# luigifcruz/radio-core

Measured on AMD Instinct MI355X. Metric: IQ Msamples/s through Tuner+WBFM at 1024 channels, higher is better.
Workload: dtype f32

## Files before the change

### radio-core_amd/csrc/fft_kernel.h

```cpp
#pragma once

#include <hip/hip_runtime.h>

#include <cstdio>
#include <cstdlib>
#include <type_traits>

#include "fft_engine.h"
#include "tile_ns.h"

namespace rcfm {
RCFM_NS_OPEN
namespace fftk {

constexpr int W = RCFM_TILE_W;
constexpr int kLogW = W == 16 ? 4 : W == 8 ? 3 : 2;
static_assert((1 << kLogW) == W, "tile width: 4, 8 or 16 lines");
constexpr int kThreads = 256 * W / 16;

__device__ __forceinline__ float2 cmul(float2 a, float2 b) {
    typedef float v2f __attribute__((ext_vector_type(2)));
    v2f A, B, D;
    A.x = a.x; A.y = a.y; B.x = b.x; B.y = b.y;
    asm("v_pk_mul_f32 %0, %1, %2 op_sel:[0,0] op_sel_hi:[0,1]" : "=v"(D) : "v"(A), "v"(B));
// ... 171 lines not shown
    dft5(v[0], v[2], v[4], v[6], v[8]);
    dft5(v[1], v[3], v[5], v[7], v[9]);
    v[3] = cmul(v[3], make_float2(0.80901699437494742410f, -0.58778525229247312917f));
    v[5] = cmul(v[5], make_float2(0.30901699437494742410f, -0.95105651629515357212f));
    v[7] = cmul(v[7], make_float2(-0.30901699437494742410f, -0.95105651629515357212f));
    v[9] = cmul(v[9], make_float2(-0.80901699437494742410f, -0.58778525229247312917f));
    dft2(v[0], v[1]);
    dft2(v[2], v[3]);
    dft2(v[4], v[5]);
    dft2(v[6], v[7]);
    dft2(v[8], v[9]);
    const float2 y0 = v[0], y5 = v[1], y1 = v[2], y6 = v[3], y2 = v[4], y7 = v[5], y3 = v[6], y8 = v[7],
                 y4 = v[8], y9 = v[9];
    v[0] = y0; v[1] = y1; v[2] = y2; v[3] = y3; v[4] = y4;
    v[5] = y5; v[6] = y6; v[7] = y7; v[8] = y8; v[9] = y9;
}

template <int R>
__device__ __forceinline__ void dif_stage(float2* tile, const float2* tw, int L, int mt, int swz) {
    const int m = mt / R;
    const int step = L / mt;
    const int nb = (L / R) * W;
    for (int e = threadIdx.x; e < nb; e += kThreads) {
        const int w = e & (W - 1);
        const int b = e / W;
        const int g = b / m;
        const int kp = b - g * m;
        const int base = g * mt + kp;
        float2 v[R];
#pragma unroll
        for (int q = 0; q < R; ++q) {
            const int row = base + q * m;
            v[q] = tile[row * W + (w ^ (swz & row & (W - 1)))];
        }
        if constexpr (R == 2) dft2(v[0], v[1]);
        if constexpr (R == 3) dft3(v[0], v[1], v[2]);
        if constexpr (R == 4) dft4(v[0], v[1], v[2], v[3]);
        if constexpr (R == 5) dft5(v[0], v[1], v[2], v[3], v[4]);
        if constexpr (R == 6) dft6(v);
        if constexpr (R == 7) dft7(v[0], v[1], v[2], v[3], v[4], v[5], v[6]);
        if constexpr (R == 8) dft8(v);
        if constexpr (R == 10) dft10(v);
        if constexpr (R > 10) dft_nat<R>(v);
        const int tstep = kp * step;
#pragma unroll
        for (int q = 1; q < R; ++q) v[q] = cmul(v[q], tw[q * tstep]);
#pragma unroll
        for (int q = 0; q < R; ++q) {
            const int row = base + q * m;
            tile[row * W + (w ^ (swz & row & (W - 1)))] = v[q];
        }
    }
}

__device__ __forceinline__ float2 big_twiddle_seed(const FftPassDev& d, unsigned e) {
    return d.coarse[e >> d.fine_bits];
}
__device__ __forceinline__ float2 big_twiddle(const FftPassDev& d, unsigned e, float2 c) {
    const float th = d.fine_step * (float)(e & ((1u << d.fine_bits) - 1u));
    const float t2 = th * th;
    const float s = th * (1.f - t2 * (1.f / 6.f) * (1.f - t2 * (1.f / 20.f)));
    const float co = 1.f - t2 * 0.5f * (1.f - t2 * (1.f / 12.f) * (1.f - t2 * (1.f / 30.f)));
    return cmul(c, make_float2(co, -s));
}
__device__ __forceinline__ float2 big_twiddle(const FftPassDev& d, unsigned e) {
    return big_twiddle(d, e, big_twiddle_seed(d, e));
}

struct LineId {
    int batch;
    int64_t o1, o2, i;
};

template <class T, class = void>
struct fetch_count { static constexpr int value = 1; };
template <class T>
struct fetch_count<T, std::void_t<decltype(T::kFetches)>> { static constexpr int value = T::kFetches; };

template <class T, class = void>
struct has_ctx : std::false_type {};
template <class T>
struct has_ctx<T, std::void_t<decltype(T::kCtx)>> : std::true_type {};

template <class LoadOp>
__device__ __forceinline__ float2 load_now(const LoadOp& load, const LineId& id, int l, int64_t base, unsigned off) {
    if constexpr (fetch_count<LoadOp>::value == 3)
        return load.post(id, l, load.fetch(id, l, base, off), load.fetch2(id, l, base, off),
                         load.fetch3(id, l, base, off));
    else if constexpr (fetch_count<LoadOp>::value == 2)
        return load.post(id, l, load.fetch(id, l, base, off), load.fetch2(id, l, base, off));
    else if constexpr (has_ctx<LoadOp>::value)
        return load.post(id, l, load.fetch(id, l, base, off), load.prepare(id));
    else
        return load.post(id, l, load.fetch(id, l, base, off));
}

template <class T, class = void>
struct has_half_zones : std::false_type {};
template <class T>
struct has_half_zones<T, std::void_t<decltype(T::kHalfZones)>> : std::bool_constant<T::kHalfZones> {};

template <class T, class = void>
struct has_aux : std::false_type {};
template <class T>
struct has_aux<T, std::void_t<decltype(T::kAux)>> : std::true_type {};

template <class StoreOp>
__device__ __forceinline__ void store_now(const StoreOp& store, const LineId& id, int k, int64_t base, unsigned off,
                                          float2 v) {
    if constexpr (has_aux<StoreOp>::value) store(id, k, base, off, v, store.fetch_aux(id, k, base, off));
    else store(id, k, base, off, v);
}

template <class LoadOp, class StoreOp>
__global__ __launch_bounds__(kThreads) void k_fft_pass(FftPassDev d, LoadOp load, StoreOp store) {
    extern __shared__ __attribute__((aligned(16))) unsigned char smem_raw[];
    const FftPass& p = d.p;
    const int L = p.L;
    float2* tile = reinterpret_cast<float2*>(smem_raw);
    float2* tw = tile + L * W;
    uint16_t* pos = reinterpret_cast<uint16_t*>(tw + L);

    const int tid = threadIdx.x;
    const int64_t tiles_inner = (p.n_inner + W - 1) / W;
    int64_t t = blockIdx.x;
    const int64_t ti = t % tiles_inner;
    t /= tiles_inner;
    LineId id;
    id.batch = blockIdx.y;
    id.o2 = t % p.n_o2;
    id.o1 = t / p.n_o2;
    const int64_t i0 = ti * W;
    const int wvalid = (int)((p.n_inner - i0) < W ? (p.n_inner - i0) : W);
    const int64_t in_base = (int64_t)id.batch * d.in_batch + id.o1 * p.in_o1 + id.o2 * p.in_o2 +
                            (p.in_t ? (i0 >> 4) * p.in_t + (i0 & 15) : i0 * p.in_i);
    const int64_t out_base = (int64_t)id.batch * d.out_batch + id.o1 * p.out_o1 + id.o2 * p.out_o2 +
                             (p.out_t ? (i0 >> 4) * p.out_t + (i0 & 15) : i0 * p.out_i);
    const int swz = p.load_along_l ? (W - 1) : 0;

    for (int e = tid; e < L; e += kThreads) {
        tw[e] = d.stage_tw[e];
        pos[e] = d.pos[e];
    }
    if (p.load_along_l) {
        for (int e = tid; e < L * W; e += kThreads) {
            const int w = e / L, l = e - w * L;
            float2 v = make_float2(0.f, 0.f);
            if (w < wvalid) {
                id.i = i0 + w;
                v = load_now(load, id, l, in_base, (unsigned)(w * p.in_i + l));
            }
            tile[l * W + (w ^ (l & (W - 1)))] = v;
        }
    } else {
        for (int e = tid; e < L * W; e += kThreads) {
            const int l = e / W, w = e & (W - 1);
            float2 v = make_float2(0.f, 0.f);
            if (w < wvalid) {
                id.i = i0 + w;
                v = load_now(load, id, l, in_base, (unsigned)(l * p.in_l + w * p.in_i));
            }
            tile[l * W + w] = v;
        }
    }
    __syncthreads();

    int mt = L;
    for (int s = 0; s < p.nstages; ++s) {
        const int r = p.radix[s];
        switch (r) {
            case 2: dif_stage<2>(tile, tw, L, mt, swz); break;
            case 3: dif_stage<3>(tile, tw, L, mt, swz); break;
            case 4: dif_stage<4>(tile, tw, L, mt, swz); break;
            case 5: dif_stage<5>(tile, tw, L, mt, swz); break;
            case 6: dif_stage<6>(tile, tw, L, mt, swz); break;
            case 7: dif_stage<7>(tile, tw, L, mt, swz); break;
            case 8: dif_stage<8>(tile, tw, L, mt, swz); break;
            case 12: dif_stage<12>(tile, tw, L, mt, swz); break;
            case 15: dif_stage<15>(tile, tw, L, mt, swz); break;
            case 16: dif_stage<16>(tile, tw, L, mt, swz); break;
            case 20: dif_stage<20>(tile, tw, L, mt, swz); break;
            case 24: dif_stage<24>(tile, tw, L, mt, swz); break;
            case 25: dif_stage<25>(tile, tw, L, mt, swz); break;
            case 32: dif_stage<32>(tile, tw, L, mt, swz); break;
            default: dif_stage<10>(tile, tw, L, mt, swz); break;
        }
        mt /= r;
        __syncthreads();
    }

    const unsigned tw_base = (unsigned)(id.o1 * p.tw_o1 + id.o2 * p.tw_o2 + i0 * p.tw_i);
    for (int e = tid; e < L * W; e += kThreads) {
        const int k = e / W, w = e & (W - 1);
        if (w >= wvalid) continue;
        const int row = pos[k];
        float2 v = tile[row * W + (w ^ (swz & row & (W - 1)))];
        if (p.has_twiddle) v = cmul(v, big_twiddle(d, (tw_base + (unsigned)w * (unsigned)p.tw_i) * (unsigned)k));
        id.i = i0 + w;
        store_now(store, id, k, out_base, (unsigned)(k * p.out_k + w * p.out_i), v);
    }
}


constexpr unsigned kXcdGroupMax = 15;
struct BlockPos {
    unsigned tile, batch;
};
struct VBlock {
    unsigned x, y, z, gx, gy, gz;
};
__device__ __forceinline__ VBlock vblock_hw() {
    return VBlock{blockIdx.x, blockIdx.y, blockIdx.z, gridDim.x, gridDim.y, gridDim.z};
}
__device__ __forceinline__ BlockPos block_pos(const VBlock& vb);
__device__ __forceinline__ BlockPos block_pos() { return block_pos(vblock_hw()); }
__device__ __forceinline__ BlockPos block_pos(const VBlock& vb) {
    const unsigned gx = vb.gx, x = vb.x, z = vb.z;
    if (gx <= kXcdGroupMax) {
        if (vb.gy == 1 && (z | 7u) < vb.gz) {
            const unsigned q = x + gx * (z & 7u);
            return BlockPos{q >> 3, (z & ~7u) + (q & 7u)};
        }
        return BlockPos{x, z};
    }
    return BlockPos{(gx & 7u) ? x : (x & 7u) * (gx >> 3) + (x >> 3), z};
}

template <int R>
__device__ __forceinline__ constexpr int dft_slot(int q) {
    if (R == 6) return (q % 3) * 2 + q / 3;
    if (R == 8) return (q % 4) * 2 + q / 4;
    if (R == 10) return (q % 5) * 2 + q / 5;
    return q;
}

__device__ __forceinline__ void dft6p(float2* v) {
    dft3(v[0], v[2], v[4]);
    dft3(v[1], v[3], v[5]);
    v[3] = cmul(v[3], make_float2(0.5f, -0.86602540378443864676f));
    v[5] = cmul(v[5], make_float2(-0.5f, -0.86602540378443864676f));
    dft2(v[0], v[1]);
    dft2(v[2], v[3]);
    dft2(v[4], v[5]);
}

__device__ __forceinline__ void dft8p(float2* v) {
    constexpr float h = 0.70710678118654752440f;
    dft4(v[0], v[2], v[4], v[6]);
    dft4(v[1], v[3], v[5], v[7]);
    v[3] = cmul(v[3], make_float2(h, -h));
    v[5] = mul_mi(v[5]);
    v[7] = cmul(v[7], make_float2(-h, -h));
    dft2(v[0], v[1]);
    dft2(v[2], v[3]);
    dft2(v[4], v[5]);
    dft2(v[6], v[7]);
}

__device__ __forceinline__ void dft10p(float2* v) {
    dft5(v[0], v[2], v[4], v[6], v[8]);
    dft5(v[1], v[3], v[5], v[7], v[9]);
    v[3] = cmul(v[3], make_float2(0.80901699437494742410f, -0.58778525229247312917f));
    v[5] = cmul(v[5], make_float2(0.30901699437494742410f, -0.95105651629515357212f));
    v[7] = cmul(v[7], make_float2(-0.30901699437494742410f, -0.95105651629515357212f));
    v[9] = cmul(v[9], make_float2(-0.80901699437494742410f, -0.58778525229247312917f));
    dft2(v[0], v[1]);
    dft2(v[2], v[3]);
    dft2(v[4], v[5]);
    dft2(v[6], v[7]);
    dft2(v[8], v[9]);
}

template <int R>
__device__ __forceinline__ void dft_p(float2* v) {
    if constexpr (R == 2) dft2(v[0], v[1]);
    if constexpr (R == 3) dft3(v[0], v[1], v[2]);
    if constexpr (R == 4) dft4(v[0], v[1], v[2], v[3]);
    if constexpr (R == 5) dft5(v[0], v[1], v[2], v[3], v[4]);
    if constexpr (R == 6) dft6p(v);
    if constexpr (R == 8) dft8p(v);
    if constexpr (R == 10) dft10p(v);
    if constexpr (R > 10 || R == 7 || R == 9) dft_nat<R>(v);
}

constexpr int kRowsPitch = W + 1;

template <bool SWZ, bool P17 = true>
__device__ __forceinline__ int lds_slot(int row, int w) {
    if (SWZ && P17) return row * (W + 1) + w;
    return SWZ ? row * W + (w ^ (row & (W - 1))) : row * W + w;
}

template <int R>
__device__ __forceinline__ void twiddle_powers(float2 w1, float2* pw) {
    pw[1] = w1;
#pragma unroll
    for (int q = 2; q < R; ++q) {
        int hb = 1;
        while (hb * 2 <= q) hb *= 2;
        pw[q] = (hb == q) ? cmul(pw[q / 2], pw[q / 2]) : cmul(pw[hb], pw[q - hb]);
    }
}

template <int L, int R, int MT, bool SWZ, int RG, bool P17 = true, bool GTW = false, int ZQ = 0>
__device__ __forceinline__ void stage_lds(float2* tile, const float2* tw, int w, int rg) {
    static_assert(ZQ == 0 || MT == L, "zero rows are declared for the first stage only");
    constexpr int m = MT / R, step = L / MT, rows = L / R, nit = (rows + RG - 1) / RG;
#pragma unroll
    for (int it = 0; it < nit; ++it) {
        const int b = rg + RG * it;
        if ((rows % RG == 0) || b < rows) {
            const int g = b / m, kp = b - g * m;
            const int base = g * MT + kp;
            float2 v[R];
            float2 pw[GTW ? R : 1];
            if constexpr (GTW) pw[0] = tw[kp * step];
#pragma unroll
            for (int q = 0; q < R; ++q) {
                if (ZQ > 0 && q >= ZQ) v[q] = make_float2(0.f, 0.f);
                else v[q] = tile[lds_slot<SWZ, P17>(base + q * m, w)];
            }
            dft_p<R>(v);
            if constexpr (GTW) {
                twiddle_powers<R>(pw[0], pw);
#pragma unroll
                for (int q = 1; q < R; ++q) v[dft_slot<R>(q)] = cmul(v[dft_slot<R>(q)], pw[q]);
            } else {
#pragma unroll
                for (int q = 1; q < R; ++q) v[dft_slot<R>(q)] = cmul(v[dft_slot<R>(q)], tw[q * kp * step]);
            }
#pragma unroll
            for (int q = 0; q < R; ++q) tile[lds_slot<SWZ, P17>(base + q * m, w)] = v[dft_slot<R>(q)];
        }
    }
}

constexpr bool big_tile_pair(int L) { return L > kFftMaxL; }
constexpr bool triple_tile(int L) { return L == 400; }

template <int L, int R0, int R1, int RL, int S>
__device__ __forceinline__ int last_stage_base(int g) {
    if constexpr (S == 2) {
        return g;
    } else if constexpr (S == 3) {
        constexpr int w1 = L / (R0 * RL);
        const int q1 = g / w1, q2 = g - q1 * w1;
        return q1 + R0 * q2;
    } else {
        constexpr int w1 = L / (R0 * RL), w2 = L / (R0 * R1 * RL);
        const int q1 = g / w1, r1 = g - q1 * w1;
        const int q2 = r1 / w2, q3 = r1 - q2 * w2;
        return q1 + R0 * (q2 + R1 * q3);
    }
}

template <int L, int R0, int R1, int R2, int R3, bool ROWS, int T, class LoadOp, class StoreOp>
__global__ __launch_bounds__(T, (big_tile_pair(L) ? 8 : triple_tile(L) ? 6 : T * 16 / W >= 512 ? 4 : 1)) void k_fft_tile(FftPassDev d, LoadOp load,
                                                                                          StoreOp store) {
    constexpr bool BIG = big_tile_pair(L) || triple_tile(L);
    constexpr int S = (R0 > 1) + (R1 > 1) + (R2 > 1) + (R3 > 1);
    static_assert(S >= 2 && R0 * R1 * R2 * R3 == L, "bad radix list");
    constexpr int RL = (S == 2) ? R1 : (S == 3) ? R2 : R3;
    constexpr int m0 = L / R0;
    constexpr int RG = T / W;
    constexpr int nit0 = (m0 + RG - 1) / RG;
    constexpr int nld = ROWS ? (L * W + T - 1) / T : nit0 * R0;
    __shared__ __attribute__((aligned(16))) float2 tile[L * (ROWS && !BIG ? kRowsPitch : W)];
    __shared__ __attribute__((aligned(16))) float2 tw_lds[BIG ? 1 : L];
    const float2* tw = BIG ? d.stage_tw : tw_lds;
    const FftPass& p = d.p;

    const int tid = threadIdx.x;
    const int w = tid & (W - 1), rg = tid >> kLogW;
    const VBlock vb = vblock_hw();
    LineId id;
    BlockPos bp = block_pos(vb);
    id.batch = bp.batch;
    unsigned o = vb.y;
    const unsigned n_o2 = (unsigned)p.n_o2;
    if (p.flat_outer) {
        const unsigned tiles_inner = ((unsigned)p.n_inner + W - 1) / W;
        o = bp.tile / tiles_inner;
        if (o >= (unsigned)(p.n_o1 * p.n_o2)) return;
        bp.tile -= o * tiles_inner;
    }
    id.o1 = n_o2 == 1 ? o : o / n_o2;
    id.o2 = n_o2 == 1 ? 0 : o - (unsigned)id.o1 * n_o2;
    const int i0 = (int)bp.tile * W;
    const int left = (int)p.n_inner - i0;
    const int wvalid = left < W ? left : W;
    const int64_t in_base = (int64_t)id.batch * d.in_batch + id.o1 * p.in_o1 + id.o2 * p.in_o2 +
                            (p.in_t ? (int64_t)(i0 >> 4) * p.in_t + (i0 & 15) : (int64_t)i0 * p.in_i);
    const int64_t out_base = (int64_t)id.batch * d.out_batch + id.o1 * p.out_o1 + id.o2 * p.out_o2 +
                             (p.out_t ? (int64_t)(i0 >> 4) * p.out_t + (i0 & 15) : (int64_t)i0);
    const unsigned in_l = (unsigned)p.in_l, in_i = (unsigned)p.in_i, out_k = (unsigned)p.out_k;

    constexpr int NF = fetch_count<LoadOp>::value;
    constexpr bool HZ = !ROWS && has_half_zones<LoadOp>::value && L % 2 == 0;
    auto zone = [](int q) -> int { return (q + 1) * m0 <= L / 2 ? 0 : (q * m0 > L / 2 ? 2 : 1); };
    float2 v[nld];
    float2 v2[NF >= 2 ? nld : 1];
    float v3[NF == 3 ? nld : 1];
    static_assert(NF <= 2 || !ROWS, "three-fetch load functors: strided passes only");
    if constexpr (ROWS) {
#pragma unroll
        for (int it = 0; it < nld; ++it) {
            int e = tid + T * it;
            if ((L * W) % T != 0) e = e < L * W ? e : 0;
            const int wl = e / L, l = e - wl * L;
            const int wc = wl < wvalid ? wl : 0;
            id.i = i0 + wc;
            v[it] = load.fetch(id, l, in_base, (unsigned)wc * in_i + (unsigned)l);
            if constexpr (NF == 2) v2[it] = load.fetch2(id, l, in_base, (unsigned)wc * in_i + (unsigned)l);
        }
    } else {
        const int wc = w < wvalid ? w : 0;
        id.i = i0 + wc;
#pragma unroll
        for (int it = 0; it < nit0; ++it) {
            int b = rg + RG * it;
            if (m0 % RG != 0) b = b < m0 ? b : 0;
#pragma unroll
            for (int q = 0; q < R0; ++q) {
                const int l = b + q * m0;
                if constexpr (HZ) {
                    const int z = zone(q);
                    if (z == 2) {
                        v[it * R0 + q] = make_float2(0.f, 0.f);
                        if constexpr (NF == 2) v2[it * R0 + q] = make_float2(0.f, 0.f);
                    } else {
                        v[it * R0 + q] = load.fetch(id, l, in_base, (unsigned)l * in_l + (unsigned)wc, z);
                        if constexpr (NF == 2)
                            v2[it * R0 + q] = load.fetch2(id, l, in_base, (unsigned)l * in_l + (unsigned)wc, z);
                    }
                } else {
                    v[it * R0 + q] = load.fetch(id, l, in_base, (unsigned)l * in_l + (unsigned)wc);
                    if constexpr (NF >= 2)
                        v2[it * R0 + q] = load.fetch2(id, l, in_base, (unsigned)l * in_l + (unsigned)wc);
                    if constexpr (NF == 3)
                        v3[it * R0 + q] = load.fetch3(id, l, in_base, (unsigned)l * in_l + (unsigned)wc);
                }
            }
        }
    }
    if constexpr (!BIG)
        for (int e = tid; e < L; e += T) tw_lds[e] = d.stage_tw[e];
    constexpr bool CTX = has_ctx<LoadOp>::value;
    static_assert(!CTX || (!ROWS && NF == 1), "load context: strided single-fetch passes only");
    auto ctx = [&] {
        if constexpr (CTX) return load.prepare(id);
        else return 0;
    }();

    constexpr int rowsL = L / RL, nitL = (rowsL + RG - 1) / RG;
    auto kbase = [](int g) -> int {
        if constexpr (S == 2) {
            return g;
        } else if constexpr (S == 3) {
            constexpr int w1 = L / (R0 * RL);
            const int q1 = g / w1, q2 = g - q1 * w1;
            return q1 + R0 * q2;
        } else {
            constexpr int w1 = L / (R0 * RL), w2 = L / (R0 * R1 * RL);
            const int q1 = g / w1, r1 = g - q1 * w1;
            const int q2 = r1 / w2, q3 = r1 - q2 * w2;
            return q1 + R0 * (q2 + R1 * q3);
        }
    };
    constexpr bool AUX = has_aux<StoreOp>::value;
    float aux[AUX ? nitL * RL : 1];
    if constexpr (AUX) {
        const int wc = w < wvalid ? w : 0;
        id.i = i0 + wc;
#pragma unroll
        for (int it = 0; it < nitL; ++it) {
            int g = rg + RG * it;
            if (rowsL % RG != 0) g = g < rowsL ? g : 0;
            const int kb = kbase(g);
#pragma unroll
            for (int q = 0; q < RL; ++q) {
                const int k = kb + (L / RL) * q;
                aux[it * RL + q] = store.fetch_aux(id, k, out_base, (unsigned)k * out_k + (unsigned)wc);
            }
        }
    }

    if constexpr (ROWS) {
#pragma unroll
        for (int it = 0; it < nld; ++it) {
            const int e = tid + T * it;
            const int wl = e / L, l = e - wl * L;
            id.i = i0 + wl;
            float2 x;
            if constexpr (NF == 2) x = load.post(id, l, v[it], v2[it]);
            else x = load.post(id, l, v[it]);
            if ((L * W) % T == 0 || e < L * W) tile[lds_slot<true, !BIG>(l, wl)] = x;
        }
        __syncthreads();
        stage_lds<L, R0, L, true, RG, !BIG, BIG>(tile, tw, w, rg);
    } else {
        if constexpr (!BIG) __syncthreads();
        id.i = i0 + (w < wvalid ? w : 0);
#pragma unroll
        for (int it = 0; it < nit0; ++it) {
            const int b = rg + RG * it;
            if ((m0 % RG == 0) || b < m0) {
                float2* x = &v[it * R0];
#pragma unroll
                for (int q = 0; q < R0; ++q) {
                    if constexpr (HZ) {
                        if constexpr (NF == 2) {
                            if (zone(q) != 2) x[q] = load.post(id, b + q * m0, x[q], v2[it * R0 + q], zone(q));
                        } else {
                            if (zone(q) != 2) x[q] = load.post(id, b + q * m0, x[q], zone(q));
                        }
                    } else if constexpr (NF == 3) x[q] = load.post(id, b + q * m0, x[q], v2[it * R0 + q], v3[it * R0 + q]);
                    else if constexpr (NF == 2) x[q] = load.post(id, b + q * m0, x[q], v2[it * R0 + q]);
                    else if constexpr (CTX) x[q] = load.post(id, b + q * m0, x[q], ctx);
                    else x[q] = load.post(id, b + q * m0, x[q]);
                }
                dft_p<R0>(x);
                if constexpr (BIG) {
                    float2 pw[R0];
                    twiddle_powers<R0>(tw[b], pw);
#pragma unroll
                    for (int q = 1; q < R0; ++q) x[dft_slot<R0>(q)] = cmul(x[dft_slot<R0>(q)], pw[q]);
                } else {
#pragma unroll
                    for (int q = 1; q < R0; ++q) x[dft_slot<R0>(q)] = cmul(x[dft_slot<R0>(q)], tw[q * b]);
                }
#pragma unroll
                for (int q = 0; q < R0; ++q) tile[lds_slot<false>(b + q * m0, w)] = x[dft_slot<R0>(q)];
            }
        }
    }
    __syncthreads();
    if constexpr (S >= 3) {
        stage_lds<L, R1, L / R0, ROWS, RG, !BIG, BIG>(tile, tw, w, rg);
        __syncthreads();
    }
    if constexpr (S >= 4) {
        stage_lds<L, R2, L / (R0 * R1), ROWS, RG, !BIG, BIG>(tile, tw, w, rg);
        __syncthreads();
    }

    const unsigned f = (unsigned)(id.o1 * p.tw_o1 + id.o2 * p.tw_o2 + (int64_t)(i0 + w) * p.tw_i);
    float2 D = make_float2(1.f, 0.f);
    constexpr bool PTW = !ROWS;
    if constexpr (PTW) D = big_twiddle(d, f * (unsigned)(L / RL));
    id.i = i0 + w;
    const bool lane_ok = w < wvalid;
#pragma unroll
    for (int it = 0; it < nitL; ++it) {
        const int g = rg + RG * it;
        if ((rowsL % RG == 0) || g < rowsL) {
            float2 x[RL];
#pragma unroll
            for (int q = 0; q < RL; ++q) x[q] = tile[lds_slot<ROWS, !BIG>(g * RL + q, w)];
            dft_p<RL>(x);
            const int kb = kbase(g);
            float2 Tw = make_float2(1.f, 0.f);
            if constexpr (PTW) Tw = big_twiddle(d, f * (unsigned)kb);
            if (lane_ok) {
#pragma unroll
                for (int q = 0; q < RL; ++q) {
                    const int k = kb + (L / RL) * q;
                    float2 y = x[dft_slot<RL>(q)];
                    if constexpr (PTW) {
                        y = cmul(y, Tw);
                        Tw = cmul(Tw, D);
                    }
                    if constexpr (AUX) store(id, k, out_base, (unsigned)k * out_k + (unsigned)w, y, aux[it * RL + q]);
                    else store(id, k, out_base, (unsigned)k * out_k + (unsigned)w, y);
                }
            }
        }
    }
}

template <class T, class = void>
struct mid_upper_rows_zero : std::false_type {};
template <class T>
struct mid_upper_rows_zero<T, std::void_t<decltype(T::kUpperRowsZero)>> : std::bool_constant<T::kUpperRowsZero> {};

template <int L, int R0, int R1, int R2, int R3, int T, class LoadOp, class MidOp, class StoreOp>
__global__ __launch_bounds__(T, (T * 16 / W >= 512 ? 4 : 1)) void k_fft_tile2(FftPassDev d1, FftPassDev d2, LoadOp load,
                                                                     MidOp mid, StoreOp store) {
    constexpr int S = (R0 > 1) + (R1 > 1) + (R2 > 1) + (R3 > 1);
    static_assert(S >= 2 && R0 * R1 * R2 * R3 == L, "bad radix list");
    constexpr int RL = (S == 2) ? R1 : (S == 3) ? R2 : R3;
    constexpr int RG = T / W;
    constexpr int nld = (L * W + T - 1) / T;
    constexpr int rowsL = L / RL, nitL = (rowsL + RG - 1) / RG;
    constexpr int kZeroQ = mid_upper_rows_zero<MidOp>::value ? (L / 2) / (L / R0) + 1 : 0;
    constexpr int kZeroFrom = kZeroQ > 0 && kZeroQ < R0 ? kZeroQ * (L / R0) : L;
    __shared__ __attribute__((aligned(16))) float2 tile[L * kRowsPitch];
    __shared__ __attribute__((aligned(16))) float2 tw[L];
    const FftPass& p1 = d1.p;
    const FftPass& p2 = d2.p;
    const int tid = threadIdx.x;
    const int w = tid & (W - 1), rg = tid >> kLogW;

    LineId id;
    const BlockPos bp = block_pos();
    id.batch = bp.batch;
    id.o1 = 0;
    id.o2 = 0;
    const int i0 = (int)bp.tile * W;
    const int left = (int)p1.n_inner - i0;
    const int wvalid = left < W ? left : W;
    const int64_t in_base = (int64_t)id.batch * d1.in_batch + (int64_t)i0 * p1.in_i;
    const int64_t mid_base = (int64_t)id.batch * d1.out_batch + i0;
    const int64_t out_base = (int64_t)id.batch * d2.out_batch + i0;
    const unsigned in_i = (unsigned)p1.in_i, mid_k = (unsigned)p1.out_k, out_k = (unsigned)p2.out_k;

    auto kbase = [](int g) -> int {
        if constexpr (S == 2) {
            return g;
        } else if constexpr (S == 3) {
            constexpr int w1 = L / (R0 * RL);
            const int q1 = g / w1, q2 = g - q1 * w1;
            return q1 + R0 * q2;
        } else {
            constexpr int w1 = L / (R0 * RL), w2 = L / (R0 * R1 * RL);
            const int q1 = g / w1, r1 = g - q1 * w1;
            const int q2 = r1 / w2, q3 = r1 - q2 * w2;
            return q1 + R0 * (q2 + R1 * q3);
        }
    };

    float2 v[nld];
#pragma unroll
    for (int it = 0; it < nld; ++it) {
        int e = tid + T * it;
        if ((L * W) % T != 0) e = e < L * W ? e : 0;
        const int wl = e / L, l = e - wl * L;
        const int wc = wl < wvalid ? wl : 0;
        id.i = i0 + wc;
        v[it] = load.fetch(id, l, in_base, (unsigned)wc * in_i + (unsigned)l);
    }
    float aux[nitL * RL];
    {
        const int wc = w < wvalid ? w : 0;
        id.i = i0 + wc;
#pragma unroll
        for (int it = 0; it < nitL; ++it) {
            int g = rg + RG * it;
            if (rowsL % RG != 0) g = g < rowsL ? g : 0;
            const int kb = kbase(g);
#pragma unroll
            for (int q = 0; q < RL; ++q) {
                const int k = kb + (L / RL) * q;
                aux[it * RL + q] = mid.fetch_aux(id, k, mid_base, (unsigned)k * mid_k + (unsigned)wc);
            }
        }
    }
    for (int e = tid; e < L; e += T) tw[e] = d1.stage_tw[e];

#pragma unroll
    for (int it = 0; it < nld; ++it) {
        const int e = tid + T * it;
        const int wl = e / L, l = e - wl * L;
        id.i = i0 + wl;
        float2 x = load.post(id, l, v[it]);
        if ((L * W) % T == 0 || e < L * W) tile[lds_slot<true>(l, wl)] = x;
    }
    lds_barrier();
    stage_lds<L, R0, L, true, RG>(tile, tw, w, rg);
    lds_barrier();
    if constexpr (S >= 3) {
        stage_lds<L, R1, L / R0, true, RG>(tile, tw, w, rg);
        lds_barrier();
    }
    if constexpr (S >= 4) {
        stage_lds<L, R2, L / (R0 * R1), true, RG>(tile, tw, w, rg);
        lds_barrier();
    }

    id.i = i0 + w;
    float2 xr[nitL * RL];
#pragma unroll
    for (int it = 0; it < nitL; ++it) {
        const int g = rg + RG * it;
        if ((rowsL % RG == 0) || g < rowsL) {
#pragma unroll
            for (int q = 0; q < RL; ++q) xr[it * RL + q] = tile[lds_slot<true>(g * RL + q, w)];
            dft_p<RL>(&xr[it * RL]);
        }
    }
    lds_barrier();
#pragma unroll
    for (int it = 0; it < nitL; ++it) {
        const int g = rg + RG * it;
        if ((rowsL % RG == 0) || g < rowsL) {
            const int kb = kbase(g);
#pragma unroll
            for (int q = 0; q < RL; ++q) {
                const int k = kb + (L / RL) * q;
                if constexpr (mid_upper_rows_zero<MidOp>::value) {
                    if ((L / RL) * q > L / 2) {
                        if ((L / RL) * q < kZeroFrom) tile[lds_slot<true>(k, w)] = make_float2(0.f, 0.f);
                        continue;
                    }
                }
                float2 y = mid(id, k, xr[it * RL + dft_slot<RL>(q)], aux[it * RL + q]);
                tile[lds_slot<true>(k, w)] = y;
            }
        }
    }
    lds_barrier();

    stage_lds<L, R0, L, true, RG, true, false, kZeroQ>(tile, tw, w, rg);
    lds_barrier();
    if constexpr (S >= 3) {
        stage_lds<L, R1, L / R0, true, RG>(tile, tw, w, rg);
        lds_barrier();
    }
    if constexpr (S >= 4) {
        stage_lds<L, R2, L / (R0 * R1), true, RG>(tile, tw, w, rg);
        lds_barrier();
    }
    const bool lane_ok = w < wvalid;
    const unsigned f = (unsigned)((int64_t)(i0 + w) * p2.tw_i);
    const float2 D = big_twiddle(d2, f * (unsigned)(L / RL));
#pragma unroll
    for (int it = 0; it < nitL; ++it) {
        const int g = rg + RG * it;
        if ((rowsL % RG == 0) || g < rowsL) {
            float2 x[RL];
#pragma unroll
            for (int q = 0; q < RL; ++q) x[q] = tile[lds_slot<true>(g * RL + q, w)];
            dft_p<RL>(x);
            const int kb = kbase(g);
            float2 Tw = big_twiddle(d2, f * (unsigned)kb);
            if (lane_ok) {
#pragma unroll
                for (int q = 0; q < RL; ++q) {
                    const int k = kb + (L / RL) * q;
                    const float2 y = cmul(x[dft_slot<RL>(q)], Tw);
                    Tw = cmul(Tw, D);
                    store(id, k, out_base, (unsigned)k * out_k + (unsigned)w, y);
                }
            }
        }
    }
}

template <int L, int R0, int R1, int R2, int R3, int T, class LoadOp, class MidOp, class StoreOp>
__global__ __launch_bounds__(T, (T * 16 / W >= 512 ? 4 : 1)) void k_fft_tile2_pair(FftPassDev d1, FftPassDev d2, LoadOp load,
                                                                          MidOp mid, StoreOp store, int count) {
    constexpr int S = (R0 > 1) + (R1 > 1) + (R2 > 1) + (R3 > 1);
    static_assert(S >= 2 && R0 * R1 * R2 * R3 == L, "bad radix list");
    constexpr int RL = (S == 2) ? R1 : (S == 3) ? R2 : R3;
    constexpr int RG = T / W;
    constexpr int nld = (L * W + T - 1) / T;
    constexpr int rowsL = L / RL, nitL = (rowsL + RG - 1) / RG;
    __shared__ __attribute__((aligned(16))) float2 tile[L * kRowsPitch];
    __shared__ __attribute__((aligned(16))) float2 tw[L];
    const FftPass& p1 = d1.p;
    const FftPass& p2 = d2.p;
    const int tid = threadIdx.x;
    const int w = tid & (W - 1), rg = tid >> kLogW;

    LineId id;
    const BlockPos bp = block_pos();
    id.batch = bp.batch;
    id.o1 = 0;
    id.o2 = 0;
    const int c0 = 2 * (int)bp.batch;
    const bool has1 = c0 + 1 < count;
    const int c1 = has1 ? c0 + 1 : c0;
    const int i0 = (int)bp.tile * W;
    const int left = (int)p1.n_inner - i0;
    const int wvalid = left < W ? left : W;
    const int64_t in_base = (int64_t)id.batch * d1.in_batch + (int64_t)i0 * p1.in_i;
    const int blk16 = mid.blk16;
    const int64_t mid_tile = blk16 ? (int64_t)(i0 >> 4) * blk16 + (i0 & 15) : (int64_t)i0;
    const int64_t mid_base0 = (int64_t)c0 * (blk16 ? mid.stride : d1.out_batch) + mid_tile;
    const int64_t mid_base1 = (int64_t)c1 * (blk16 ? mid.stride : d1.out_batch) + mid_tile;
    const int64_t out_base0 = (int64_t)c0 * d2.out_batch + i0;
    const int64_t out_base1 = (int64_t)c1 * d2.out_batch + i0;
    const unsigned in_i = (unsigned)p1.in_i, mid_k = blk16 ? 16u : (unsigned)p1.out_k, out_k = (unsigned)p2.out_k;
    const int wc = w < wvalid ? w : 0;

    auto lane_off = [&](int it) -> unsigned {
        int g = rg + RG * it;
        if (rowsL % RG != 0) g = g < rowsL ? g : 0;
        return (unsigned)last_stage_base<L, R0, R1, RL, S>(g) * mid_k + (unsigned)wc;
    };
    auto q_off = [&](int q) -> int64_t { return (int64_t)((L / RL) * q) * mid_k; };

    float2 v[nld];
#pragma unroll
    for (int it = 0; it < nld; ++it) {
        int e = tid + T * it;
        if ((L * W) % T != 0) e = e < L * W ? e : 0;
        const int wl = e / L, l = e - wl * L;
        const int wcl = wl < wvalid ? wl : 0;
        id.i = i0 + wcl;
        v[it] = load.fetch(id, l, in_base, (unsigned)wcl * in_i + (unsigned)l);
    }
    for (int e = tid; e < L; e += T) tw[e] = d1.stage_tw[e];
#pragma unroll
    for (int it = 0; it < nld; ++it) {
        const int e = tid + T * it;
        const int wl = e / L, l = e - wl * L;
        id.i = i0 + wl;
        const float2 x = load.post(id, l, v[it]);
        if ((L * W) % T == 0 || e < L * W) tile[lds_slot<true>(l, wl)] = x;
    }
    lds_barrier();
    stage_lds<L, R0, L, true, RG>(tile, tw, w, rg);
    lds_barrier();
    if constexpr (S >= 3) {
        stage_lds<L, R1, L / R0, true, RG>(tile, tw, w, rg);
        lds_barrier();
    }
    if constexpr (S >= 4) {
        stage_lds<L, R2, L / (R0 * R1), true, RG>(tile, tw, w, rg);
        lds_barrier();
    }

    using In0 = decltype(mid.fetch0(mid_base0, mid_base1, 0u));
    In0 a0[nitL * RL];
#pragma unroll
    for (int it = 0; it < nitL; ++it)
#pragma unroll
        for (int q = 0; q < RL; ++q)
            a0[it * RL + q] = mid.fetch0(mid_base0 + q_off(q), mid_base1 + q_off(q), lane_off(it));

    id.i = i0 + w;
    using Keep = typename MidOp::Keep;
    float2 u0[nitL * RL];
    Keep keep[nitL * RL];
#pragma unroll
    for (int it = 0; it < nitL; ++it) {
        const int g = rg + RG * it;
        if ((rowsL % RG == 0) || g < rowsL) {
            float2 x[RL];
#pragma unroll
            for (int q = 0; q < RL; ++q) x[q] = tile[lds_slot<true>(g * RL + q, w)];
            dft_p<RL>(x);
#pragma unroll
            for (int q = 0; q < RL; ++q)
                u0[it * RL + q] = mid.first(x[dft_slot<RL>(q)], a0[it * RL + q], keep[it * RL + q]);
        }
        __builtin_amdgcn_sched_barrier(0);
    }
    lds_barrier();
#pragma unroll
    for (int it = 0; it < nitL; ++it) {
        const int g = rg + RG * it;
        if ((rowsL % RG == 0) || g < rowsL) {
            const int kb = last_stage_base<L, R0, R1, RL, S>(g);
#pragma unroll
            for (int q = 0; q < RL; ++q) tile[lds_slot<true>(kb + (L / RL) * q, w)] = u0[it * RL + q];
        }
    }
    lds_barrier();

    const unsigned f = (unsigned)((int64_t)(i0 + w) * p2.tw_i);
    const float2 D = big_twiddle(d2, f * (unsigned)(L / RL));
    const bool lane_ok = w < wvalid;
    auto second_transform = [&](int64_t out_base) {
        stage_lds<L, R0, L, true, RG>(tile, tw, w, rg);
        lds_barrier();
        if constexpr (S >= 3) {
            stage_lds<L, R1, L / R0, true, RG>(tile, tw, w, rg);
            lds_barrier();
        }
        if constexpr (S >= 4) {
            stage_lds<L, R2, L / (R0 * R1), true, RG>(tile, tw, w, rg);
            lds_barrier();
        }
#pragma unroll
        for (int it = 0; it < nitL; ++it) {
            const int g = rg + RG * it;
            if ((rowsL % RG == 0) || g < rowsL) {
                float2 x[RL];
#pragma unroll
                for (int q = 0; q < RL; ++q) x[q] = tile[lds_slot<true>(g * RL + q, w)];
                dft_p<RL>(x);
                const int kb = last_stage_base<L, R0, R1, RL, S>(g);
                float2 Tw = big_twiddle(d2, f * (unsigned)kb);
                if (lane_ok) {
#pragma unroll
                    for (int q = 0; q < RL; ++q) {
                        const int k = kb + (L / RL) * q;
                        const float2 y = cmul(x[dft_slot<RL>(q)], Tw);
                        Tw = cmul(Tw, D);
                        store(id, k, out_base, (unsigned)k * out_k + (unsigned)w, y);
                    }
                }
            }
        }
    };

    float a1[nitL * RL];
#pragma unroll
    for (int it = 0; it < nitL; ++it)
#pragma unroll
        for (int q = 0; q < RL; ++q) a1[it * RL + q] = mid.fetch1(mid_base1 + q_off(q), lane_off(it));

    second_transform(out_base0);
    if (!has1) return;
    lds_barrier();
#pragma unroll
    for (int it = 0; it < nitL; ++it) {
        const int g = rg + RG * it;
        if ((rowsL % RG == 0) || g < rowsL) {
            const int kb = last_stage_base<L, R0, R1, RL, S>(g);
#pragma unroll
            for (int q = 0; q < RL; ++q) {
                const int k = kb + (L / RL) * q;
                tile[lds_slot<true>(k, w)] = mid.second(keep[it * RL + q], a1[it * RL + q]);
            }
        }
    }
    lds_barrier();
    second_transform(out_base1);
}

template <int L, int R0, int R1, int R2, int R3, int L2, int Q0, int Q1, int Q2, int T, class LoadOp, class WinOp, class StoreOp>
__global__ __launch_bounds__(T, (T * 16 / W >= 512 ? 4 : 1)) void k_fft_tile2_decim(FftPassDev d1, FftPassDev d2, LoadOp load,
                                                                           WinOp win, StoreOp store) {
    constexpr int S = (R0 > 1) + (R1 > 1) + (R2 > 1) + (R3 > 1);
    static_assert(S >= 2 && R0 * R1 * R2 * R3 == L, "bad radix list");
    constexpr int S2 = (Q0 > 1) + (Q1 > 1) + (Q2 > 1);
    static_assert(S2 >= 2 && Q0 * Q1 * Q2 == L2 && L2 % 2 == 0 && L2 < L, "bad short transform");
    constexpr int RL = (S == 2) ? R1 : (S == 3) ? R2 : R3;
    constexpr int QL = (S2 == 2) ? Q1 : Q2;
    constexpr int RG = T / W;
    constexpr int nld = (L * W + T - 1) / T;
    constexpr int rowsL = L / RL, nitL = (rowsL + RG - 1) / RG;
    constexpr int rows2 = L2 / QL;
    static_assert(rows2 <= RG, "short transform: one sweep");
    constexpr bool REG = S == 2 && nitL == 1 && Q0 == 4 && L2 == 4 * rowsL && RL >= 5 && L % L2 == 0;
    constexpr int nwin = REG ? 4 : (L2 * W + T - 1) / T;
    __shared__ __attribute__((aligned(16))) float2 tile[L * kRowsPitch];
    __shared__ __attribute__((aligned(16))) float2 tw[L];
    const FftPass& p1 = d1.p;
    const FftPass& p2 = d2.p;
    const int tid = threadIdx.x;
    const int w = tid & (W - 1), rg = tid >> kLogW;

    LineId id;
    const BlockPos bp = block_pos();
    id.batch = bp.batch;
    id.o1 = 0;
    id.o2 = 0;
    const int i0 = (int)bp.tile * W;
    const int left = (int)p1.n_inner - i0;
    const int wvalid = left < W ? left : W;
    const int64_t in_base = (int64_t)id.batch * d1.in_batch + (int64_t)i0 * p1.in_i;
    const int64_t out_base = (int64_t)id.batch * d2.out_batch + i0;
    const unsigned in_i = (unsigned)p1.in_i, out_k = (unsigned)p2.out_k;

    float2 v[nld];
#pragma unroll
    for (int it = 0; it < nld; ++it) {
        int e = tid + T * it;
        if ((L * W) % T != 0) e = e < L * W ? e : 0;
        const int wl = e / L, l = e - wl * L;
        const int wcl = wl < wvalid ? wl : 0;
        id.i = i0 + wcl;
        v[it] = load.fetch(id, l, in_base, (unsigned)wcl * in_i + (unsigned)l);
    }
    float wgt[nwin];
    if constexpr (REG) {
        const int g = rg < rowsL ? rg : 0;
#pragma unroll
        for (int q = 0; q < 4; ++q) wgt[q] = win.weight(id, g + rowsL * q, i0 + (w < wvalid ? w : 0));
    } else {
#pragma unroll
        for (int it = 0; it < nwin; ++it) {
            int e = tid + T * it;
            if ((L2 * W) % T != 0) e = e < L2 * W ? e : 0;
            const int wl = e & (W - 1);
            wgt[it] = win.weight(id, e >> kLogW, i0 + (wl < wvalid ? wl : 0));
        }
    }
    const unsigned f = (unsigned)((int64_t)(i0 + w) * p2.tw_i);
    const int kb2 = last_stage_base<L2, Q0, Q1, QL, S2>(rg < rows2 ? rg : 0);
    const float2 seedD = big_twiddle_seed(d2, f * (unsigned)rows2);
    const float2 seedT = big_twiddle_seed(d2, f * (unsigned)kb2);
    float2 tw2 = make_float2(0.f, 0.f);
    if constexpr (REG && S2 == 3) {
        static_assert(L2 <= T, "short stage table: one entry per thread");
        tw2 = d2.stage_tw[tid < L2 ? tid : 0];
    }
    for (int e = tid; e < L; e += T) tw[e] = d1.stage_tw[e];
#pragma unroll
    for (int it = 0; it < nld; ++it) {
        const int e = tid + T * it;
        const int wl = e / L, l = e - wl * L;
        id.i = i0 + wl;
        const float2 x = load.post(id, l, v[it]);
        if ((L * W) % T == 0 || e < L * W) tile[lds_slot<true>(l, wl)] = x;
    }
    lds_barrier();
    stage_lds<L, R0, L, true, RG>(tile, tw, w, rg);
    lds_barrier();
    if constexpr (S >= 3) {
        stage_lds<L, R1, L / R0, true, RG>(tile, tw, w, rg);
        lds_barrier();
    }
    if constexpr (S >= 4) {
        stage_lds<L, R2, L / (R0 * R1), true, RG>(tile, tw, w, rg);
        lds_barrier();
    }

    float2 xr[nitL * RL];
#pragma unroll
    for (int it = 0; it < nitL; ++it) {
        const int g = rg + RG * it;
        if ((rowsL % RG == 0) || g < rowsL) {
#pragma unroll
            for (int q = 0; q < RL; ++q) xr[it * RL + q] = tile[lds_slot<true>(g * RL + q, w)];
            dft_p<RL>(&xr[it * RL]);
        }
    }
    if constexpr (REG) {
        float2 y[4];
        if (rg < rowsL) {
            y[0] = xr[dft_slot<RL>(0)];
            y[1] = xr[dft_slot<RL>(1)];
            y[2] = xr[dft_slot<RL>(RL - 2)];
            y[3] = xr[dft_slot<RL>(RL - 1)];
            const bool first = rg == 0 && i0 + w == 0;
            if (first) y[2] = cadd(y[2], xr[dft_slot<RL>(2)]);
#pragma unroll
            for (int q = 0; q < 4; ++q) y[q] = make_float2(y[q].x * wgt[q], y[q].y * wgt[q]);
            if (first) {
                id.i = 0;
                win.dc_bin(id, y[0]);
            }
#pragma unroll
            for (int q = 0; q < 4; ++q) y[q] = make_float2(y[q].y, y[q].x);
            dft4(y[0], y[1], y[2], y[3]);
#pragma unroll
            for (int q = 1; q < 4; ++q) y[q] = cmul(y[q], tw[(L / L2) * q * rg]);
        }
        lds_barrier();
        if (rg < rowsL) {
#pragma unroll
            for (int q = 0; q < 4; ++q) tile[lds_slot<true>(rg + rowsL * q, w)] = y[q];
        }
        if constexpr (S2 == 3) {
            if (tid < L2) tw[tid] = tw2;
        }
        lds_barrier();
    } else {
        lds_barrier();
#pragma unroll
        for (int it = 0; it < nitL; ++it) {
            const int g = rg + RG * it;
            if ((rowsL % RG == 0) || g < rowsL) {
                const int kb = last_stage_base<L, R0, R1, RL, S>(g);
#pragma unroll
                for (int q = 0; q < RL; ++q) {
                    if ((L / RL) * q > L2 / 2 && (L / RL) * (q + 1) <= L - L2 / 2) continue;
                    const int k = kb + (L / RL) * q;
                    int l = -1;
                    if (k < L2 / 2) l = k;
                    else if (k >= L - L2 / 2) l = k - (L - L2);
                    else if (k == L2 / 2) l = L2;
                    if (l >= 0) tile[lds_slot<true>(l, w)] = xr[it * RL + dft_slot<RL>(q)];
                }
            }
        }
        for (int e = tid; e < L2; e += T) tw[e] = d2.stage_tw[e];
        lds_barrier();

#pragma unroll
        for (int it = 0; it < nwin; ++it) {
            const int e = tid + T * it;
            if ((L2 * W) % T == 0 || e < L2 * W) {
                const int l = e >> kLogW, wl = e & (W - 1);
                float2 x = tile[lds_slot<true>(l, wl)];
                if (l == L2 / 2 && i0 + wl == 0) {
                    const float2 y = tile[lds_slot<true>(L2, wl)];
                    x = make_float2(x.x + y.x, x.y + y.y);
                }
                x = make_float2(x.x * wgt[it], x.y * wgt[it]);
                if (l == 0 && i0 + wl == 0) {
                    id.i = 0;
                    win.dc_bin(id, x);
                }
                tile[lds_slot<true>(l, wl)] = make_float2(x.y, x.x);
            }
        }
        lds_barrier();

        stage_lds<L2, Q0, L2, true, RG>(tile, tw, w, rg);
        lds_barrier();
    }
    if constexpr (S2 == 3) {
        stage_lds<L2, Q1, L2 / Q0, true, RG>(tile, tw, w, rg);
        lds_barrier();
    }
    id.i = i0 + w;
    if (rg < rows2) {
        float2 x[QL];
#pragma unroll
        for (int q = 0; q < QL; ++q) x[q] = tile[lds_slot<true>(rg * QL + q, w)];
        dft_p<QL>(x);
        const float2 D = big_twiddle(d2, f * (unsigned)rows2, seedD);
        float2 Tw = big_twiddle(d2, f * (unsigned)kb2, seedT);
        if (w < wvalid) {
#pragma unroll
            for (int q = 0; q < QL; ++q) {
                const int k = kb2 + rows2 * q;
                const float2 y = cmul(x[dft_slot<QL>(q)], Tw);
                Tw = cmul(Tw, D);
                store(id, k, out_base, (unsigned)k * out_k + (unsigned)w, y);
            }
        }
    }
}


__device__ __forceinline__ float2 stream_load(const float2* p) { return *p; }

__device__ __forceinline__ void stream_store(float2* p, float2 v) {
    if constexpr (W == 16) {
        using v2 = __attribute__((ext_vector_type(2))) float;
        v2 t;
        t.x = v.x;
        t.y = v.y;
        __builtin_nontemporal_store(t, reinterpret_cast<v2*>(p));
    } else {
        *p = v;
    }
}

template <bool SWAP>
struct LoadPlainT {
    const float2* in;
    __device__ __forceinline__ float2 fetch(const LineId&, int, int64_t base, unsigned off) const {
        return stream_load(in + base + off);
    }
    __device__ __forceinline__ float2 post(const LineId&, int, float2 v) const {
        return SWAP ? make_float2(v.y, v.x) : v;
    }
};

template <bool SWAP>
struct StorePlainT {
    float2* out;
    float scale;
    __device__ __forceinline__ void operator()(const LineId&, int, int64_t base, unsigned off, float2 v) const {
        stream_store(out + base + off,
                     SWAP ? make_float2(v.y * scale, v.x * scale) : make_float2(v.x * scale, v.y * scale));
    }
};

struct StoreRowWindow {
    float2* out;
    float scale;
    int n_o1, n_o2, lo, hi;
    int64_t n = 0;
    int halo = 0;
    int sc1_straddle = 0;
    __device__ __forceinline__ void operator()(const LineId& id, int k, int64_t base, unsigned off, float2 v) const {
        const int row = (int)id.o1 + n_o1 * ((int)id.o2 + n_o2 * k);
        const bool keep = lo <= hi ? (row >= lo && row <= hi) : (row >= lo || row <= hi);
        if (!keep) return;
        const float2 y = make_float2(v.x * scale, v.y * scale);
        const int64_t g = base + off;
        const bool straddle = sc1_straddle &&
                              ((reinterpret_cast<uintptr_t>(out + g) - ((uintptr_t)((int)id.i & (W - 1)) << 3)) & 127u) != 0;
        if (straddle) asm volatile("global_store_dwordx2 %0, %1, off sc1" : : "v"(out + g), "v"(y) : "memory");
        else stream_store(out + g, y);
        if (halo > 0) {
            if (g < halo) out[n + g] = y;
            else if (g >= n - halo) out[g - n] = y;
        }
    }
};

}
RCFM_NS_CLOSE
}
namespace rcfm {
RCFM_NS_OPEN
namespace fftk {

#define RCFM_FFT_LONG_TABLE3(X) X(480, 10, 8, 6, 1) X(500, 10, 10, 5, 1)
#define RCFM_FFT_LONG_TABLE(X) X(480, 24, 20, 1, 1) X(500, 25, 20, 1, 1)
#ifndef RCFM_R640
#define RCFM_R640 10, 8, 8, 1
#endif
#ifndef RCFM_R600
#define RCFM_R600 10, 10, 6, 1
#endif
#define RCFM_FFT_BIG_X_(X, LEN, ...) X(LEN, __VA_ARGS__)
#define RCFM_FFT_BIG_LENGTHS(X) RCFM_FFT_BIG_X_(X, 600, RCFM_R600) X(625, 5, 5, 5, 5) RCFM_FFT_BIG_X_(X, 640, RCFM_R640)
#define RCFM_FFT_LENGTHS_(X, LONGT) \
    X(75, 5, 5, 3, 1)            \
    X(80, 10, 8, 1, 1)           \
    X(100, 10, 10, 1, 1)         \
    X(120, 12, 10, 1, 1)         \
    X(125, 5, 5, 5, 1)           \
    X(128, 8, 8, 2, 1)           \
    X(150, 15, 10, 1, 1)         \
    X(160, 16, 10, 1, 1)         \
    X(192, 16, 12, 1, 1)         \
    X(200, 20, 10, 1, 1)         \
    X(240, 24, 10, 1, 1)         \
    X(250, 25, 10, 1, 1)         \
    X(256, 16, 16, 1, 1)         \
    X(300, 20, 15, 1, 1)         \
    X(320, 10, 8, 4, 1)          \
    X(375, 5, 5, 5, 3)           \
    X(384, 8, 8, 6, 1)           \
    X(400, 20, 20, 1, 1)         \
    LONGT(X)                     \
    X(512, 8, 8, 8, 1)
#define RCFM_FFT_FAST_LENGTHS(X) RCFM_FFT_LENGTHS_(X, RCFM_FFT_LONG_TABLE)
// ... 160 lines not shown
```

Before: 34970.

## Fuse second FFT's first stage into registers with reversed radix order

```diff
diff --git a/radio-core_amd/csrc/fft_kernel.h b/radio-core_amd/csrc/fft_kernel.h
--- a/radio-core_amd/csrc/fft_kernel.h
+++ b/radio-core_amd/csrc/fft_kernel.h
@@ -497,9 +497,8 @@
     }
 }
 
-template <int L, int R, int MT, bool SWZ, int RG, bool P17 = true, bool GTW = false, int ZQ = 0>
+template <int L, int R, int MT, bool SWZ, int RG, bool P17 = true, bool GTW = false>
 __device__ __forceinline__ void stage_lds(float2* tile, const float2* tw, int w, int rg) {
-    static_assert(ZQ == 0 || MT == L, "zero rows are declared for the first stage only");
     constexpr int m = MT / R, step = L / MT, rows = L / R, nit = (rows + RG - 1) / RG;
 #pragma unroll
     for (int it = 0; it < nit; ++it) {
@@ -511,10 +510,7 @@
             float2 pw[GTW ? R : 1];
             if constexpr (GTW) pw[0] = tw[kp * step];
 #pragma unroll
-            for (int q = 0; q < R; ++q) {
-                if (ZQ > 0 && q >= ZQ) v[q] = make_float2(0.f, 0.f);
-                else v[q] = tile[lds_slot<SWZ, P17>(base + q * m, w)];
-            }
+            for (int q = 0; q < R; ++q) v[q] = tile[lds_slot<SWZ, P17>(base + q * m, w)];
             dft_p<R>(v);
             if constexpr (GTW) {
                 twiddle_powers<R>(pw[0], pw);
@@ -773,6 +769,25 @@
     }
 }
 
+#ifndef RCFM_PAIR_SWAP_TAIL
+#define RCFM_PAIR_SWAP_TAIL 0
+#endif
+template <int R0, int R1, int R2, int R3>
+struct reversed_radices {
+    static constexpr int S = (R0 > 1) + (R1 > 1) + (R2 > 1) + (R3 > 1);
+    static constexpr int Q0 = (S == 2) ? R1 : (S == 3) ? R2 : R3;
+    static constexpr int Q1 = (S == 2) ? R0 : (S == 3) ? R1 : R2;
+    static constexpr int Q2 = (S == 3) ? R0 : (S == 4) ? R1 : 1;
+    static constexpr int QL = R0;
+};
+
+template <int R>
+__device__ __forceinline__ void first_stage_regs(float2* y, const float2* tw, int b) {
+    dft_p<R>(y);
+#pragma unroll
+    for (int q = 1; q < R; ++q) y[dft_slot<R>(q)] = cmul(y[dft_slot<R>(q)], tw[q * b]);
+}
+
 template <class T, class = void>
 struct mid_upper_rows_zero : std::false_type {};
 template <class T>
@@ -787,8 +802,10 @@
     constexpr int RG = T / W;
     constexpr int nld = (L * W + T - 1) / T;
     constexpr int rowsL = L / RL, nitL = (rowsL + RG - 1) / RG;
-    constexpr int kZeroQ = mid_upper_rows_zero<MidOp>::value ? (L / 2) / (L / R0) + 1 : 0;
-    constexpr int kZeroFrom = kZeroQ > 0 && kZeroQ < R0 ? kZeroQ * (L / R0) : L;
+    using Rev = reversed_radices<R0, R1, R2, R3>;
+    constexpr int Q0 = Rev::Q0, Q1 = Rev::Q1, Q2 = Rev::Q2, QL = Rev::QL;
+    static_assert(Q0 == RL, "the second transform starts with the first one's last radix");
+    constexpr int rows2 = L / QL, nit2 = (rows2 + RG - 1) / RG;
     __shared__ __attribute__((aligned(16))) float2 tile[L * kRowsPitch];
     __shared__ __attribute__((aligned(16))) float2 tw[L];
     const FftPass& p1 = d1.p;
@@ -881,6 +898,17 @@
 #pragma unroll
             for (int q = 0; q < RL; ++q) xr[it * RL + q] = tile[lds_slot<true>(g * RL + q, w)];
             dft_p<RL>(&xr[it * RL]);
+            const int kb = kbase(g);
+            float2 y[RL];
+#pragma unroll
+            for (int q = 0; q < RL; ++q) {
+                const int k = kb + (L / RL) * q;
+                if (mid_upper_rows_zero<MidOp>::value && (L / RL) * q > L / 2) y[q] = make_float2(0.f, 0.f);
+                else y[q] = mid(id, k, xr[it * RL + dft_slot<RL>(q)], aux[it * RL + q]);
+            }
+            first_stage_regs<RL>(y, tw, kb);
+#pragma unroll
+            for (int q = 0; q < RL; ++q) xr[it * RL + q] = y[dft_slot<RL>(q)];
         }
     }
     lds_barrier();
@@ -890,49 +918,37 @@
         if ((rowsL % RG == 0) || g < rowsL) {
             const int kb = kbase(g);
 #pragma unroll
-            for (int q = 0; q < RL; ++q) {
-                const int k = kb + (L / RL) * q;
-                if constexpr (mid_upper_rows_zero<MidOp>::value) {
-                    if ((L / RL) * q > L / 2) {
-                        if ((L / RL) * q < kZeroFrom) tile[lds_slot<true>(k, w)] = make_float2(0.f, 0.f);
-                        continue;
-                    }
-                }
-                float2 y = mid(id, k, xr[it * RL + dft_slot<RL>(q)], aux[it * RL + q]);
-                tile[lds_slot<true>(k, w)] = y;
-            }
+            for (int q = 0; q < RL; ++q) tile[lds_slot<true>(kb + (L / RL) * q, w)] = xr[it * RL + q];
         }
     }
     lds_barrier();
 
-    stage_lds<L, R0, L, true, RG, true, false, kZeroQ>(tile, tw, w, rg);
-    lds_barrier();
     if constexpr (S >= 3) {
-        stage_lds<L, R1, L / R0, true, RG>(tile, tw, w, rg);
+        stage_lds<L, Q1, L / Q0, true, RG>(tile, tw, w, rg);
         lds_barrier();
     }
     if constexpr (S >= 4) {
-        stage_lds<L, R2, L / (R0 * R1), true, RG>(tile, tw, w, rg);
+        stage_lds<L, Q2, L / (Q0 * Q1), true, RG>(tile, tw, w, rg);
         lds_barrier();
     }
     const bool lane_ok = w < wvalid;
     const unsigned f = (unsigned)((int64_t)(i0 + w) * p2.tw_i);
-    const float2 D = big_twiddle(d2, f * (unsigned)(L / RL));
-#pragma unroll
-    for (int it = 0; it < nitL; ++it) {
+    const float2 D = big_twiddle(d2, f * (unsigned)(L / QL));
+#pragma unroll
+    for (int it = 0; it < nit2; ++it) {
         const int g = rg + RG * it;
-        if ((rowsL % RG == 0) || g < rowsL) {
-            float2 x[RL];
-#pragma unroll
-            for (int q = 0; q < RL; ++q) x[q] = tile[lds_slot<true>(g * RL + q, w)];
-            dft_p<RL>(x);
-            const int kb = kbase(g);
+        if ((rows2 % RG == 0) || g < rows2) {
+            float2 x[QL];
+#pragma unroll
+            for (int q = 0; q < QL; ++q) x[q] = tile[lds_slot<true>(g * QL + q, w)];
+            dft_p<QL>(x);
+            const int kb = last_stage_base<L, Q0, Q1, QL, S>(g);
             float2 Tw = big_twiddle(d2, f * (unsigned)kb);
             if (lane_ok) {
 #pragma unroll
-                for (int q = 0; q < RL; ++q) {
-                    const int k = kb + (L / RL) * q;
-                    const float2 y = cmul(x[dft_slot<RL>(q)], Tw);
+                for (int q = 0; q < QL; ++q) {
+                    const int k = kb + (L / QL) * q;
+                    const float2 y = cmul(x[dft_slot<QL>(q)], Tw);
                     Tw = cmul(Tw, D);
                     store(id, k, out_base, (unsigned)k * out_k + (unsigned)w, y);
                 }
@@ -950,6 +966,11 @@
     constexpr int RG = T / W;
     constexpr int nld = (L * W + T - 1) / T;
     constexpr int rowsL = L / RL, nitL = (rowsL + RG - 1) / RG;
+    using Rev = reversed_radices<R0, R1, R2, R3>;
+    constexpr bool kSwapTail = RCFM_PAIR_SWAP_TAIL && S == 3;
+    constexpr int Q0 = Rev::Q0, Q1 = kSwapTail ? Rev::QL : Rev::Q1, Q2 = Rev::Q2, QL = kSwapTail ? Rev::Q1 : Rev::QL;
+    static_assert(Q0 == RL, "the second transform starts with the first one's last radix");
+    constexpr int rows2 = L / QL, nit2 = (rows2 + RG - 1) / RG;
     __shared__ __attribute__((aligned(16))) float2 tile[L * kRowsPitch];
     __shared__ __attribute__((aligned(16))) float2 tw[L];
     const FftPass& p1 = d1.p;
@@ -1036,9 +1057,12 @@
 #pragma unroll
             for (int q = 0; q < RL; ++q) x[q] = tile[lds_slot<true>(g * RL + q, w)];
             dft_p<RL>(x);
-#pragma unroll
-            for (int q = 0; q < RL; ++q)
-                u0[it * RL + q] = mid.first(x[dft_slot<RL>(q)], a0[it * RL + q], keep[it * RL + q]);
+            float2 y[RL];
+#pragma unroll
+            for (int q = 0; q < RL; ++q) y[q] = mid.first(x[dft_slot<RL>(q)], a0[it * RL + q], keep[it * RL + q]);
+            first_stage_regs<RL>(y, tw, last_stage_base<L, R0, R1, RL, S>(g));
+#pragma unroll
+            for (int q = 0; q < RL; ++q) u0[it * RL + q] = y[dft_slot<RL>(q)];
         }
         __builtin_amdgcn_sched_barrier(0);
     }
@@ -1055,34 +1079,32 @@
     lds_barrier();
 
     const unsigned f = (unsigned)((int64_t)(i0 + w) * p2.tw_i);
-    const float2 D = big_twiddle(d2, f * (unsigned)(L / RL));
+    const float2 D = big_twiddle(d2, f * (unsigned)(L / QL));
     const bool lane_ok = w < wvalid;
     auto second_transform = [&](int64_t out_base) {
-        stage_lds<L, R0, L, true, RG>(tile, tw, w, rg);
-        lds_barrier();
         if constexpr (S >= 3) {
-            stage_lds<L, R1, L / R0, true, RG>(tile, tw, w, rg);
+            stage_lds<L, Q1, L / Q0, true, RG>(tile, tw, w, rg);
             lds_barrier();
         }
         if constexpr (S >= 4) {
-            stage_lds<L, R2, L / (R0 * R1), true, RG>(tile, tw, w, rg);
+            stage_lds<L, Q2, L / (Q0 * Q1), true, RG>(tile, tw, w, rg);
             lds_barrier();
         }
 #pragma unroll
-        for (int it = 0; it < nitL; ++it) {
+        for (int it = 0; it < nit2; ++it) {
             const int g = rg + RG * it;
-            if ((rowsL % RG == 0) || g < rowsL) {
-                float2 x[RL];
-#pragma unroll
-                for (int q = 0; q < RL; ++q) x[q] = tile[lds_slot<true>(g * RL + q, w)];
-                dft_p<RL>(x);
-                const int kb = last_stage_base<L, R0, R1, RL, S>(g);
+            if ((rows2 % RG == 0) || g < rows2) {
+                float2 x[QL];
+#pragma unroll
+                for (int q = 0; q < QL; ++q) x[q] = tile[lds_slot<true>(g * QL + q, w)];
+                dft_p<QL>(x);
+                const int kb = last_stage_base<L, Q0, Q1, QL, S>(g);
                 float2 Tw = big_twiddle(d2, f * (unsigned)kb);
                 if (lane_ok) {
 #pragma unroll
-                    for (int q = 0; q < RL; ++q) {
-                        const int k = kb + (L / RL) * q;
-                        const float2 y = cmul(x[dft_slot<RL>(q)], Tw);
+                    for (int q = 0; q < QL; ++q) {
+                        const int k = kb + (L / QL) * q;
+                        const float2 y = cmul(x[dft_slot<QL>(q)], Tw);
                         Tw = cmul(Tw, D);
                         store(id, k, out_base, (unsigned)k * out_k + (unsigned)w, y);
                     }
@@ -1105,11 +1127,12 @@
         const int g = rg + RG * it;
         if ((rowsL % RG == 0) || g < rowsL) {
             const int kb = last_stage_base<L, R0, R1, RL, S>(g);
-#pragma unroll
-            for (int q = 0; q < RL; ++q) {
-                const int k = kb + (L / RL) * q;
-                tile[lds_slot<true>(k, w)] = mid.second(keep[it * RL + q], a1[it * RL + q]);
-            }
+            float2 y[RL];
+#pragma unroll
+            for (int q = 0; q < RL; ++q) y[q] = mid.second(keep[it * RL + q], a1[it * RL + q]);
+            first_stage_regs<RL>(y, tw, kb);
+#pragma unroll
+            for (int q = 0; q < RL; ++q) tile[lds_slot<true>(kb + (L / RL) * q, w)] = y[dft_slot<RL>(q)];
         }
     }
     lds_barrier();
```

Measured after the change: 35220 (median of 6 runs). About the same (+0.7%).
